# cvg/limap

Hardware: NVIDIA H100
Metric: 3D line candidates triangulated+scored/sec (higher is better)
Workload: dtype f64

## Files before the change

### limap_b200/csrc/engine.cu

```cuda
#include "engine.cuh"
#include <cub/device/device_radix_sort.cuh>
#include <cub/device/device_scan.cuh>
#include <algorithm>
#include <cstdlib>
#include <memory>
#include <set>

M3h quat_to_R(const double q_in[4]) {
  double n = std::sqrt(q_in[0] * q_in[0] + q_in[1] * q_in[1] + q_in[2] * q_in[2] + q_in[3] * q_in[3]);
  double q[4];
  if (n == 0) { q[0] = 1; q[1] = q_in[1]; q[2] = q_in[2]; q[3] = q_in[3]; }
  else for (int i = 0; i < 4; ++i) q[i] = q_in[i] / n;
  const double w = q[0], x = q[1], y = q[2], z = q[3];
  const double tx = 2 * x, ty = 2 * y, tz = 2 * z, twx = tx * w, twy = ty * w, twz = tz * w;
  const double txx = tx * x, txy = ty * x, txz = tz * x, tyy = ty * y, tyz = tz * y, tzz = tz * z;
  M3h R;
  R.m[0] = 1 - (tyy + tzz); R.m[1] = txy - twz; R.m[2] = txz + twy;
  R.m[3] = txy + twz; R.m[4] = 1 - (txx + tzz); R.m[5] = tyz - twx;
  R.m[6] = txz - twy; R.m[7] = tyz + twx; R.m[8] = 1 - (txx + tyy);
  return R;
}

void make_view(int model_id, const double *kv, const double *qv, const double *t, lm::ViewD &d) {
  const double fx = kv[0], fy = kv[1], cx = kv[2], cy = kv[3];
// ... 622 lines not shown
  p.ranges_flag = c->ranges_flag;
  for (int i = 0; i < 3; ++i) { p.rlo[i] = c->rlo[i]; p.rhi[i] = c->rhi[i]; }
  p.l2d = to_dev<double>(g.linker2d);
  {
    lm_linker_config l3 = g.linker3d;
    l3.use_angle = 1; l3.use_overlap = 0; l3.use_perp = 0; l3.use_innerseg = 0; l3.use_scaleinv = 1;
    p.l3d = to_dev<double>(l3);
  }
  {
    const double kPi = 3.14159265358979323846;
    const double t3 = p.l3d.th_angle, t2 = p.l2d.th_angle;
    p.cos_th3d_f = (t3 >= 90.0) ? -1.0f : (float)(std::cos(t3 * kPi / 180.0) - 4e-6);
    const double c2 = (t2 >= 90.0) ? 0.0 : std::cos(t2 * kPi / 180.0);
    p.cos2_th2d = c2 * c2;
    p.th_perp2_2d = p.l2d.th_perp * p.l2d.th_perp;
    const double ta = p.line_tri_angle_threshold, tsn = p.sensitivity_threshold;
    p.tri_poly_ok = (ta > 0.0 && ta < 90.0);
    p.sens_poly_ok = (tsn > 0.0 && tsn < 90.0);
    p.sin2_tri = std::sin(ta * kPi / 180.0) * std::sin(ta * kPi / 180.0);
    p.sin2_sens = std::sin(tsn * kPi / 180.0) * std::sin(tsn * kPi / 180.0);
    p.fast_forms = (p.l2d.use_innerseg || getenv("LIMAP_B200_REFERENCE_FORMS")) ? 0 : 1;
    p.inv_sig_a3 = 1.0 / (p.l3d.th_angle * p.l3d.mult);
    p.inv_sig_s3 = 1.0 / (p.l3d.th_scaleinv * p.l3d.mult);
    p.inv_sig_a2 = 1.0 / (p.l2d.th_angle * p.l2d.mult);
    p.inv_sig_p2 = 1.0 / (p.l2d.th_perp * p.l2d.mult);
    p.q_cut3 = -2.0 * std::log(p.l3d.score_th) * (1.0 + 1e-9);
    p.q_cut3_lo = -2.0 * std::log(p.l3d.score_th) * (1.0 - 1e-9);
    p.q_cut2 = -2.0 * std::log(p.l2d.score_th) * (1.0 + 1e-9);
    p.q_cut2_lo = -2.0 * std::log(p.l2d.score_th) * (1.0 - 1e-9);
    p.inv_smart_den2 = 1.0 / (p.l2d.th_smartoverlap - p.l2d.th_overlap);
  }
  int nbits = 1;
  while (((int64_t)1 << nbits) < c->n_nodes) ++nbits;
  c->sorted_key = c->d_key2.as<uint32_t>();
  c->sorted_val = c->d_val2.as<uint32_t>();
  p.row_ng = c->sorted_val;
  const int n_groups = exhaustive ? 1 : (int)std::max<int64_t>(1, std::min<int64_t>(c->pipeline_groups, n_rows >> 16));
  c->node_kernel_ms_acc = 0;
  int bg0 = 0, gv0 = vb;
  const int64_t n_shard_nodes = c->node_end - c->node_begin;
  if (!c->outside_shard_clean && (c->node_begin > 0 || c->node_end < c->n_nodes)) {
    if (c->node_begin > 0) {
      CU(cudaMemsetAsync(c->d_nodes.p, 0, sizeof(lm::NodeRecord) * c->node_begin, s));
      CU(cudaMemsetAsync(c->d_node_row_off.p, 0, 4 * c->node_begin, s));
    }
    if (c->node_end < c->n_nodes) {
      CU(cudaMemsetAsync(c->d_nodes.as<lm::NodeRecord>() + c->node_end, 0, sizeof(lm::NodeRecord) * (c->n_nodes - c->node_end), s));
      CU(cudaMemsetAsync(c->d_node_row_off.as<uint32_t>() + c->node_end + 1, 0, 4 * (c->n_nodes - c->node_end), s));
    }
    c->outside_shard_clean = true;
  }
  const bool fast_kernel = p.fast_forms && !p.use_endpoints_triangulation;
  const size_t smem_limit = (size_t)std::max(0, c->max_smem_optin - 1024);
  int cap = c->cap_hint > 0 ? c->cap_hint : 224;
  if (exhaustive && c->cap_hint == 0) {
    int64_t mr = 0, cur = 0;
    int cur_src = -1;
    for (int i = 0; i < nb; ++i) {
      if (blk[i].src_view != cur_src) { cur_src = blk[i].src_view; cur = 0; }
      cur += c->line_off[blk[i].ng_view + 1] - c->line_off[blk[i].ng_view];
      mr = std::max(mr, cur);
    }
    if (mr * ns > 65535) return fail(LM_ERR_INVALID, "more than 65535 candidates possible for one 2D line");
    cap = 32;
    while (cap < mr * ns) cap += 32;
  }
  while ((int)c->evk.size() < 2 * n_groups) {
    cudaEvent_t e;
    CU(cudaEventCreate(&e));
    c->evk.push_back(e);
  }
  while ((int)c->evp.size() < n_groups) {
    cudaEvent_t e;
    CU(cudaEventCreateWithFlags(&e, cudaEventDisableTiming));
    c->evp.push_back(e);
  }
  std::vector<int> group_has_kernel(n_groups, 0);
  CU(c->d_nvalid.ensure(4 * (n_shard_nodes + 2)));
  CU(c->d_local_off.ensure(4 * (n_shard_nodes + 2)));
  CU(c->d_edge_off.ensure(4 * (n_shard_nodes + 2)));
  CU(c->d_edge_ng.ensure(4 * std::max<int64_t>(n_rows * ns, 1)));
  for (int g = 0; g < n_groups; ++g) {
    int bg1 = nb, gv1 = ve;
    if (g + 1 < n_groups) {
      const double tg = (g + 1.0) / n_groups;
      const int64_t target = (int64_t)((double)n_rows * (tg * tg * (3.0 - 2.0 * tg)));
      bg1 = bg0;
      while (bg1 < nb && row_off[bg1] < target) ++bg1;
      while (bg1 < nb && bg1 > 0 && blk[bg1].src_view == blk[bg1 - 1].src_view) ++bg1;
      gv1 = (bg1 < nb) ? blk[bg1].src_view : ve;
    }
    const int64_t rb = row_off[bg0], re = row_off[bg1];
    const int64_t node_lo = c->line_off[gv0], node_hi = c->line_off[gv1];
    if (!exhaustive && re > rb) {
      int64_t need = 0;
      for (int b2 = bg0; b2 < bg1; ++b2) need = std::max(need, pair_off[b2] + blk[b2].n_rows);
      for (const auto &ch : c->chunks)
        if (ch.row_end >= need) { CU(cudaStreamWaitEvent(sp, ch.ev, 0)); break; }
    }
    unsigned int *d_max_rows = c->d_scalars.as<unsigned int>() + 16 + g;
    if (re > rb) {
      if (exhaustive)
        lm::launch_expand_exhaustive(c->d_blk_row_off.as<int64_t>(), c->d_blk_src.as<int32_t>(), c->d_blk_ng.as<int32_t>(),
                                     nb, c->d_line_off.as<int64_t>(), n_rows, c->d_key.as<uint32_t>(),
                                     c->d_val.as<uint32_t>(), sp);
      else
        lm::launch_expand_rows(c->d_pairs.as<int32_t>(), c->d_blk_row_off.as<int64_t>(), c->d_blk_src.as<int32_t>(),
                               c->d_blk_ng.as<int32_t>(), c->d_blk_pair_off.as<int64_t>(), nb,
                               c->d_line_off.as<int64_t>(), rb, re, c->d_key.as<uint32_t>(), c->d_val.as<uint32_t>(),
                               d_err, sp);
      ++launches;
      cub::DoubleBuffer<uint32_t> dk(c->d_key.as<uint32_t>() + rb, c->d_key2.as<uint32_t>() + rb);
      cub::DoubleBuffer<uint32_t> dv(c->d_val.as<uint32_t>() + rb, c->d_val2.as<uint32_t>() + rb);
      CU(cub_call(c->d_sort_tmp, [&](void *t, size_t &b) {
        return cub::DeviceRadixSort::SortPairs(t, b, dk, dv, (int)(re - rb), 0, nbits, sp);
      }));
      launches += (nbits + 7) / 8 + 1;
      if (dk.Current() != c->d_key2.as<uint32_t>() + rb) {
// ... 20 lines not shown
      p.cap = cap;
      grid = (int)std::min<int64_t>(n_group_nodes, (int64_t)c->sm_count * 4);
      p.slab_stride = (int64_t)((smem + 255) / 256 * 256);
      CU(c->d_slab.ensure((size_t)p.slab_stride * std::max(grid, 1)));
      p.slab = c->d_slab.as<char>();
      smem = 0;
    }
    if (n_group_nodes > 0) {
      CU(cudaEventRecord(c->evk[2 * g], s));
      CU(lm::launch_tri_node_kernel(p, grid, 128, smem, s));
      CU(cudaEventRecord(c->evk[2 * g + 1], s));
      group_has_kernel[g] = 1;
      ++launches;
      {
        cudaStream_t so = c->out_stream;
        CU(cudaStreamWaitEvent(so, c->evk[2 * g + 1], 0));
        uint32_t *nv = c->d_nvalid.as<uint32_t>() + (node_lo - c->node_begin);
        lm::launch_extract_nvalid(p.nodes, node_lo, n_group_nodes, nv, so);
        CU(cub_call(c->d_scan_tmp, [&](void *t, size_t &b) {
          return cub::DeviceScan::ExclusiveSum(t, b, nv, c->d_local_off.as<uint32_t>(), (int)(n_group_nodes + 1), so);
        }));
        lm::launch_group_edges(p.row_state, p.row_ng, p.node_row_off, c->d_local_off.as<uint32_t>(),
                               c->d_scalars.as<unsigned int>() + 80, g, c->node_begin, node_lo, n_group_nodes, ns,
                               c->d_edge_off.as<uint32_t>(), c->d_edge_ng.as<uint32_t>(), so);
        launches += 4;
      }
      if (c->node_sink) {
        CU(cudaMemcpyAsync(c->node_sink + sizeof(lm::NodeRecord) * node_lo, c->d_nodes.as<lm::NodeRecord>() + node_lo,
                           sizeof(lm::NodeRecord) * n_group_nodes, cudaMemcpyDeviceToHost, c->out_stream));
      }
    }
    bg0 = bg1;
    gv0 = gv1;
  }
  p.node_begin = c->node_begin;
  p.node_end = c->node_end;
  CU(cudaGetLastError());
  CU(cudaEventRecord(c->ev_run_begin, c->out_stream));
  CU(cudaStreamWaitEvent(s, c->ev_run_begin, 0));
  CU(cudaEventRecord(c->ev1, s));
  unsigned int *hs = c->h_pin;
  CU(cudaMemcpyAsync(hs, c->d_scalars.p, 512, cudaMemcpyDeviceToHost, s));
  CU(cudaStreamSynchronize(s));
  CU(cudaStreamSynchronize(c->copy_stream));
  CU(cudaStreamSynchronize(c->out_stream));
  c->stats.n_kernel_launches += launches;
  if (hs[1] == 1)
    return fail(LM_ERR_INVALID, "IndexError! Out-of-index matches exist (line_id >= number of lines of the image). "
                                "Please make sure you are reusing the correct descriptors and matches.");
  if (hs[1] == 2) return fail(LM_ERR_INVALID, "IndexError! Out-of-index neighbor line id in matches.");
  int max_rows_all = 0;
  for (int g = 0; g < n_groups; ++g) max_rows_all = std::max(max_rows_all, (int)hs[16 + g]);
  if ((int64_t)max_rows_all * ns > 65535) return fail(LM_ERR_INVALID, "more than 65535 candidates possible for one 2D line");
  int need_cap = 32;
  while (need_cap < max_rows_all * ns) need_cap += 32;
  c->cap_hint = need_cap;
  if (hs[2] != 0) {
    if (c->run_retry) { c->run_retry = 0; return fail(LM_ERR_STATE, "node staging overflow after resizing"); }
    c->run_retry = 1;
    const int rc2 = lm_tri_run(c);
    c->run_retry = 0;
    return rc2;
  }
  float ms = 0;
  CU(cudaEventElapsedTime(&ms, c->ev0, c->ev1));
  for (int g = 0; g < n_groups; ++g)
    if (group_has_kernel[g]) {
      float msk = 0;
      CU(cudaEventElapsedTime(&msk, c->evk[2 * g], c->evk[2 * g + 1]));
      c->node_kernel_ms_acc += msk;
    }
  c->stats.max_rows_per_node = max_rows_all;
  c->stats.last_node_kernel_ms = c->node_kernel_ms_acc;
  const unsigned long long *cnt = reinterpret_cast<const unsigned long long *>(hs + 4);
  c->stats.n_rows = n_rows;
  c->stats.n_candidates = (int64_t)cnt[0];
  c->stats.n_valid_edges = (int64_t)cnt[1];
  c->stats.n_pairs_gated = (int64_t)cnt[2];
  c->stats.n_pairs_exact = (int64_t)cnt[3];
  c->stats.last_run_ms = ms;
  c->ran = true;
  return LM_OK;
}

int lm_tri_get_stats(lm_ctx *c, lm_tri_stats *out) {
  if (!c || !out) return fail(LM_ERR_INVALID, "NULL argument");
  *out = c->stats;
  return LM_OK;
}

int lm_tri_get_best(lm_ctx *c, int32_t img_id, double *out_line, int32_t *out_ng, int32_t *out_ncand) {
  if (!c) return fail(LM_ERR_INVALID, "ctx is NULL");
  int rc = ensure_ran(c);
  if (rc) return rc;
  if ((rc = fetch_nodes(c))) return rc;
  auto it = c->id2view.find(img_id);
  if (it == c->id2view.end()) return fail(LM_ERR_INVALID, "unknown image id");
  const int v = it->second;
  for (int64_t n = c->line_off[v]; n < c->line_off[v + 1]; ++n) {
    const lm::NodeRecord &r = c->h_nodes[n];
    const int64_t l = n - c->line_off[v];
    for (int k = 0; k < 9; ++k) out_line[10 * l + k] = r.line[k];
    out_line[10 * l + 9] = r.score;
    out_ng[2 * l] = r.n_cand ? c->img_ids[r.ng_view] : 0;
    out_ng[2 * l + 1] = r.ng_line;
    if (out_ncand) out_ncand[l] = r.n_cand;
  }
  return LM_OK;
}
// ... 162 lines not shown
```

### limap_b200/csrc/tri_kernels.cu

```cuda
#include "tri_kernels.cuh"
#include <algorithm>
#include <cstdio>

namespace lm {

#ifndef LM_TRI_MIN_BLOCKS
#define LM_TRI_MIN_BLOCKS 4
#endif
static constexpr int kThreads = 128;
static constexpr int kWarps = kThreads / 32;
#ifndef LM_TRI_TMA
#define LM_TRI_TMA 0
#endif
#ifndef LM_KFLUSH
#define LM_KFLUSH 64
#endif
static constexpr int kFlush = LM_KFLUSH;
static constexpr int kListExtra = kFlush + 32;
static constexpr int kCandBytes = 17 * 8 + 48 + 8;

size_t tri_smem_bytes(int cap, bool fast) {
  if (fast) return (size_t)cap * (20 * 8 + kWarps * 8 + 32 + 8 + 4 + 2 + kWarps * 2);
  return (size_t)cap * kCandBytes + (size_t)kWarps * 2 * (cap + kListExtra) * 4 + (size_t)kWarps * cap * 2;
}

struct __align__(16) GateRec {
  float dx, dy, dz, lims2;
  float sx, sy, sz, lime2;
  float ex, ey, ez, pad;
};

struct __align__(16) GateRecF {
  float dx, dy, dz, lam_e;
  float lam_s;
  float lim_s, lim_e;
  int img;
};

struct Slab {
  double *sx, *sy, *sz, *ex, *ey, *ez, *dx, *dy, *dz, *zs, *ze, *unc, *q0, *q1, *q2, *q3, *score;
  double *izs2, *ize2, *inb;
  GateRec *gate;
  uint32_t *ng, *row;
  uint32_t *list;
  uint16_t *list0;
  GateRecF *gatef;
  float *slam;
  uint16_t *sidx;
  double *psc;
  uint16_t *pent;
  LM_D void carve(char *base, int cap, bool fast) {
    if (fast) { carve_fast(base, cap); return; }
    gatef = nullptr; slam = nullptr; sidx = nullptr; psc = nullptr; pent = nullptr;
    double *d = reinterpret_cast<double *>(base);
    sx = d; sy = sx + cap; sz = sy + cap; ex = sz + cap; ey = ex + cap; ez = ey + cap;
    dx = ez + cap; dy = dx + cap; dz = dy + cap; zs = dz + cap; ze = zs + cap; unc = ze + cap;
    q0 = unc + cap; q1 = q0 + cap; q2 = q1 + cap; q3 = q2 + cap; score = q3 + cap;
    double *nx = score + cap;
    izs2 = ize2 = inb = nullptr;
    if (fast) { izs2 = nx; ize2 = izs2 + cap; inb = ize2 + cap; nx = inb + cap; }
    gate = reinterpret_cast<GateRec *>(nx);
    ng = reinterpret_cast<uint32_t *>(gate + cap);
    row = ng + cap;
    list = row + cap;
    list0 = reinterpret_cast<uint16_t *>(list + (size_t)kWarps * (fast ? 1 : 2) * (cap + kListExtra));
  }
  LM_D void carve_fast(char *base, int cap) {
    double *d = reinterpret_cast<double *>(base);
    sx = d; sy = sx + cap; sz = sy + cap; ex = sz + cap; ey = ex + cap; ez = ey + cap;
    dx = ez + cap; dy = dx + cap; dz = dy + cap; zs = dz + cap; ze = zs + cap; unc = ze + cap;
    q0 = unc + cap; q1 = q0 + cap; q2 = q1 + cap; q3 = q2 + cap; score = q3 + cap;
    izs2 = score + cap; ize2 = izs2 + cap; inb = ize2 + cap;
    psc = inb + cap;
    gatef = reinterpret_cast<GateRecF *>(psc + (size_t)kWarps * cap);
    ng = reinterpret_cast<uint32_t *>(gatef + cap);
    row = ng + cap;
    slam = reinterpret_cast<float *>(row + cap);
    sidx = reinterpret_cast<uint16_t *>(slam + cap);
    pent = sidx + cap;
    gate = nullptr; list = nullptr; list0 = nullptr;
  }
};

LM_D uint32_t smem_u32(const void *p) { return (uint32_t)__cvta_generic_to_shared(p); }
LM_D void mbar_init(unsigned long long *bar, int count) {
  asm volatile("mbarrier.init.shared::cta.b64 [%0], %1;" ::"r"(smem_u32(bar)), "r"(count) : "memory");
  asm volatile("fence.mbarrier_init.release.cluster;" ::: "memory");
}
LM_D void mbar_arrive_expect_tx(unsigned long long *bar, uint32_t bytes) {
  asm volatile("mbarrier.arrive.expect_tx.shared::cta.b64 _, [%0], %1;" ::"r"(smem_u32(bar)), "r"(bytes) : "memory");
}
LM_D void bulk_copy_g2s(void *dst_smem, const void *src_gmem, uint32_t bytes, unsigned long long *bar) {
  asm volatile("cp.async.bulk.shared::cluster.global.mbarrier::complete_tx::bytes [%0], [%1], %2, [%3];" ::"r"(smem_u32(dst_smem)),
               "l"(src_gmem), "r"(bytes), "r"(smem_u32(bar))
               : "memory");
}
LM_D void mbar_wait(unsigned long long *bar, uint32_t parity) {
  uint32_t done = 0;
  while (!done) {
    asm volatile("{\n .reg .pred p;\n mbarrier.try_wait.parity.shared::cta.b64 p, [%1], %2;\n selp.u32 %0, 1, 0, p;\n}"
                 : "=r"(done)
                 : "r"(smem_u32(bar)), "r"(parity)
                 : "memory");
  }
}

struct Cand {
  vec3<double> s, e;
  double zs, ze, unc;
  double lam_s, lam_e;
};

LM_D double4 ld_seg(const double4 *p) {
  const double2 a = __ldg(reinterpret_cast<const double2 *>(p));
  const double2 b = __ldg(reinterpret_cast<const double2 *>(p) + 1);
  return make_double4(a.x, a.y, b.x, b.y);
}
LM_D double deg_from_cos_abs(double c) { return acos(fabs(c)) * consts<double>::rad2deg(); }

LM_D bool triangulate_point(const ViewD &v1, const ViewD &v2, vec3<double> n1e, vec3<double> n2e, vec3<double> C1,
                            vec3<double> C2, vec3<double> &out) {
  double a00 = dot(n1e, n1e), a01 = -dot(n1e, n2e), a10 = -dot(n2e, n1e), a11 = dot(n2e, n2e);
  double b0 = dot(n1e, C2 - C1), b1 = dot(n2e, C1 - C2);
  double r0, r1;
  if (a00 >= a11) {
    double l10 = a10 / a00, d1 = a11 - l10 * a01, y1 = b1 - l10 * b0;
    r1 = y1 / d1;
    r0 = (b0 - a01 * r1) / a00;
  } else {
    double l01 = a01 / a11, d0 = a00 - l01 * a10, y0 = b0 - l01 * b1;
    r0 = y0 / d0;
    r1 = (b1 - a10 * r0) / a11;
  }
// ... 191 lines not shown
  return true;
}

LM_D double pair_score(const TriParams &p, const seg<vec3<double>> &Li, vec3<double> di, double zsi, double zei,
                       const Slab &sl, int j, uint32_t vj) {
  const LinkerDev<double> &c3 = p.l3d;
  double score3 = 1.0;
  {
    double cs = fabs(di.x * sl.dx[j] + di.y * sl.dy[j] + di.z * sl.dz[j]);
    double angle = acos(cs) * consts<double>::rad2deg();
    score3 = smin(score3, thresh0(expscore(angle, c3.th_angle * c3.mult), c3.score_th));
    if (score3 < c3.score_th) return 0.0;
    vec3<double> sj = mk3(sl.sx[j], sl.sy[j], sl.sz[j]), ej = mk3(sl.ex[j], sl.ey[j], sl.ez[j]);
    double ds = norm(Li.s - sj), de = norm(Li.e - ej);
    double dist = smax(ds / (zsi + consts<double>::eps()), de / (zei + consts<double>::eps()));
    score3 = smin(score3, thresh0(expscore(dist, c3.th_scaleinv * c3.mult), c3.score_th));
    if (score3 == 0.0) return 0.0;
  }
  const ViewD &v = p.views[vj];
  seg<vec2<double>> a, b;
  a.s = dehom(proj_h(v.P, Li.s));
  a.e = dehom(proj_h(v.P, Li.e));
  b.s = mk2(sl.q0[j], sl.q1[j]);
  b.e = mk2(sl.q2[j], sl.q3[j]);
  double score2 = linker_score<double, vec2<double>>(p.l2d, a, b, 1.0, false, 0.0, 0.0);
  if (score2 == 0.0) return 0.0;
  return smin(score3, score2);
}

LM_D double asin2_over_t(double t) {
  double r = 0.017069849551821746;
  r = fma(r, t, 0.019089950090498877);
  r = fma(r, t, 0.02154247840073658);
  r = fma(r, t, 0.02456910759753428);
  r = fma(r, t, 0.028377319275152094);
  r = fma(r, t, 0.03328204112517838);
  r = fma(r, t, 0.03978243978243978);
  r = fma(r, t, 0.04871319157033443);
  r = fma(r, t, 0.06156806156806157);
  r = fma(r, t, 0.08126984126984127);
  r = fma(r, t, 0.11428571428571428);
  r = fma(r, t, 0.17777777777777778);
  r = fma(r, t, 0.3333333333333333);
  r = fma(r, t, 1.0);
  return r;
}
LM_D double angle2_deg(double t, double abs_cos) {
  const double k = consts<double>::rad2deg();
  if (t <= 0.0625) return t * asin2_over_t(t) * (k * k);
  const double a = acos(abs_cos) * k;
  return a * a;
}

LM_D double pair_score_fast(const TriParams &p, const Slab &sl, int i, int j, uint32_t vj) {
  const double EPS = consts<double>::eps();
  const LinkerDev<double> &c3 = p.l3d;
  const LinkerDev<double> &c2 = p.l2d;
  const vec3<double> si = mk3(sl.sx[i], sl.sy[i], sl.sz[i]), ei = mk3(sl.ex[i], sl.ey[i], sl.ez[i]);
  double Q = 0.0;
  {
    const vec3<double> di = mk3(sl.dx[i], sl.dy[i], sl.dz[i]), dj = mk3(sl.dx[j], sl.dy[j], sl.dz[j]);
    const vec3<double> cr = mk3(__dmul_rn(di.y, dj.z) - __dmul_rn(di.z, dj.y), __dmul_rn(di.z, dj.x) - __dmul_rn(di.x, dj.z),
                                __dmul_rn(di.x, dj.y) - __dmul_rn(di.y, dj.x));
    double a2 = angle2_deg(dot(cr, cr), fabs(dot(di, dj)));
    if (!(dot(di, di) * dot(dj, dj) > 0.5)) a2 = 8100.0;
    if (a2 == a2) Q = a2 * (p.inv_sig_a3 * p.inv_sig_a3);
    const vec3<double> ds = si - mk3(sl.sx[j], sl.sy[j], sl.sz[j]), de = ei - mk3(sl.ex[j], sl.ey[j], sl.ez[j]);
    const double r2 = fmax(dot(ds, ds) * sl.izs2[i], dot(de, de) * sl.ize2[i]);
    Q = fmax(Q, r2 * p.inv_sig_s3 * p.inv_sig_s3);
    if (Q > p.q_cut3) return 0.0;
  }
  const ViewD &v = p.views[vj];
  const vec3<double> hs = proj_h(v.P, si), he = proj_h(v.P, ei);
  const double ws = 1.0 / (hs.z + EPS), we = 1.0 / (he.z + EPS);
  const vec2<double> as = mk2(hs.x * ws, hs.y * ws), ae = mk2(he.x * we, he.y * we);
  const vec2<double> bs = mk2(sl.q0[j], sl.q1[j]), be = mk2(sl.q2[j], sl.q3[j]);
  const vec2<double> va = ae - as, vb = be - bs;
  const double na2 = dot(va, va), nb2 = dot(vb, vb);
  const double dab = dot(va, vb);
  const double ina = 1.0 / na2, inb = sl.inb[j];
  double Q2 = 0.0;
  double ang2 = 0.0;
  if (c2.use_angle) {
    if (dab * dab < p.cos2_th2d * na2 * nb2 * (1.0 - 1e-9)) return 0.0;
    if (na2 > 0.0 && nb2 > 0.0) {
      const double cr = va.x * vb.y - va.y * vb.x;
      const double t = cr * cr * (ina * inb);
      ang2 = angle2_deg(t, (t <= 0.0625) ? 0.0 : fabs(dab) / sqrt(na2 * nb2));
    } else {
      ang2 = 8100.0;
    }
    if (ang2 == ang2) Q2 = ang2 * (p.inv_sig_a2 * p.inv_sig_a2);
  }
  double bio = 0.0;
  if (c2.use_overlap) {
    double p1 = dot(as - bs, vb) * inb, p2 = dot(ae - bs, vb) * inb;
    if (p1 > p2) { const double t = p1; p1 = p2; p2 = t; }
    const double o1 = smin(p2, 1.0) - smax(p1, 0.0);
    double r1 = dot(bs - as, va) * ina, r2 = dot(be - as, va) * ina;
    if (r1 > r2) { const double t = r1; r1 = r2; r2 = t; }
    const double o2 = smin(r2, 1.0) - smax(r1, 0.0);
    bio = smax(o1, o2);
    if (!(bio > c2.th_overlap)) return 0.0;
  }
  if (c2.use_angle && c2.use_overlap && c2.use_smartangle && bio < c2.th_smartoverlap) {
    double ratio = (c2.th_smartoverlap - bio) * p.inv_smart_den2;
    ratio = smin(ratio, 1.0);
    const double sig = (c2.th_angle - ratio * (c2.th_angle - c2.th_smartangle)) * c2.mult;
    if (ang2 == ang2) Q2 = fmax(Q2, ang2 / (sig * sig));
  }
  if (c2.use_perp) {
    const vec2<double> d0 = as - bs, d1 = ae - bs, d2 = bs - as, d3 = be - as;
    const double t0 = dot(d0, vb), t1 = dot(d1, vb), t2 = dot(d2, va), t3 = dot(d3, va);
    double m = fmax(dot(d0, d0) - t0 * t0 * inb, 0.0);
    m = fmax(m, dot(d1, d1) - t1 * t1 * inb);
    m = fmax(m, dot(d2, d2) - t2 * t2 * ina);
    m = fmax(m, dot(d3, d3) - t3 * t3 * ina);
    Q2 = fmax(Q2, m * p.inv_sig_p2 * p.inv_sig_p2);
  }
  if (Q2 > p.q_cut2) return 0.0;
  if (Q < p.q_cut3_lo && Q2 < p.q_cut2_lo) return exp(-fmax(Q, Q2) * 0.5);
  const double e3 = exp(-Q * 0.5), e2 = exp(-Q2 * 0.5);
  if (e3 < c3.score_th || e2 < c2.score_th) return 0.0;
  return smin(e3, e2);
}


LM_D bool gate3d(const GateRec &r, const GateRec *g, float cos_th) {
  const float4 a = *reinterpret_cast<const float4 *>(&g->dx);
  const float cs = fabsf(r.dx * a.x + r.dy * a.y + r.dz * a.z);
  if (cs < cos_th) return false;
  const float4 b = *reinterpret_cast<const float4 *>(&g->sx);
  const float ax = r.sx - b.x, ay = r.sy - b.y, az = r.sz - b.z;
  if (ax * ax + ay * ay + az * az > r.lims2) return false;
  const float4 c = *reinterpret_cast<const float4 *>(&g->ex);
  const float bx = r.ex - c.x, by = r.ey - c.y, bz = r.ez - c.z;
  return !(bx * bx + by * by + bz * bz > r.lime2);
}

LM_D bool gate3d_rest(const GateRec &r, const GateRec *g, float cos_th) {
  const float4 a = *reinterpret_cast<const float4 *>(&g->dx);
  if (fabsf(r.dx * a.x + r.dy * a.y + r.dz * a.z) < cos_th) return false;
  const float4 c = *reinterpret_cast<const float4 *>(&g->ex);
  const float bx = r.ex - c.x, by = r.ey - c.y, bz = r.ez - c.z;
  return !(bx * bx + by * by + bz * bz > r.lime2);
}

LM_D bool gate2d(const TriParams &p, const seg<vec3<double>> &Li, const Slab &sl, int j, uint32_t vj) {
  const LinkerDev<double> &c = p.l2d;
  const ViewD &v = p.views[vj];
  const vec2<double> as = dehom(proj_h(v.P, Li.s)), ae = dehom(proj_h(v.P, Li.e));
  const vec2<double> bs = mk2(sl.q0[j], sl.q1[j]), be = mk2(sl.q2[j], sl.q3[j]);
  const vec2<double> va = ae - as, vb = be - bs;
  const double na2 = dot(va, va), nb2 = dot(vb, vb);
  const double REL = 1e-9;
  if (c.use_angle) {
    const double d = dot(va, vb);
    if (d * d < p.cos2_th2d * na2 * nb2 * (1.0 - REL)) return false;
  }
  if (c.use_overlap) {
    double p1 = dot(as - bs, vb) / nb2, p2 = dot(ae - bs, vb) / nb2;
    if (p1 > p2) { const double t = p1; p1 = p2; p2 = t; }
    const double o1 = smin(p2, 1.0) - smax(p1, 0.0);
    double r1 = dot(bs - as, va) / na2, r2 = dot(be - as, va) / na2;
    if (r1 > r2) { const double t = r1; r1 = r2; r2 = t; }
    const double o2 = smin(r2, 1.0) - smax(r1, 0.0);
    const double bio = smax(o1, o2);
    if (bio < c.th_overlap - REL * (1.0 + fabs(c.th_overlap))) return false;
  }
  if (c.use_perp) {
    const vec2<double> d0 = as - bs, d1 = ae - bs, d2 = bs - as, d3 = be - as;
    const double t0 = dot(d0, vb), t1 = dot(d1, vb), t2 = dot(d2, va), t3 = dot(d3, va);
    double m = dot(d0, d0) - t0 * t0 / nb2;
    m = fmax(m, dot(d1, d1) - t1 * t1 / nb2);
    m = fmax(m, dot(d2, d2) - t2 * t2 / na2);
    m = fmax(m, dot(d3, d3) - t3 * t3 / na2);
    if (m > p.th_perp2_2d * (1.0 + REL) + REL) return false;
  }
  return true;
}

template <bool SLAB, bool VP, bool FAST>
__global__ void __launch_bounds__(kThreads, LM_TRI_MIN_BLOCKS) tri_node_kernel(const __grid_constant__ TriParams p) {
  constexpr int NS = VP ? 3 : 1;
  extern __shared__ __align__(16) unsigned char smem_raw[];
  __shared__ int s_wtot[kWarps];
  __shared__ int s_nvalid;
  __shared__ int s_next_row;
  __shared__ __align__(8) unsigned long long s_mbar;
  uint32_t mbar_parity = 0;
  if constexpr (FAST && !SLAB && (LM_TRI_TMA || VP)) {
    if (threadIdx.x == 0) mbar_init(&s_mbar, 1);
    __syncthreads();
  }
  const int tid = threadIdx.x, lane = tid & 31, warp = tid >> 5;
  const unsigned lt_mask = (1u << lane) - 1u;
  Slab sl;
  if (SLAB) sl.carve(p.slab + (int64_t)blockIdx.x * p.slab_stride, p.cap, FAST);
  else sl.carve(reinterpret_cast<char *>(smem_raw), p.cap, FAST);
  uint32_t *list1 = FAST ? nullptr : sl.list + (size_t)(warp * 2) * (p.cap + kListExtra);
  uint32_t *list2 = FAST ? nullptr : list1 + p.cap + kListExtra;
  uint16_t *list0 = FAST ? nullptr : sl.list0 + (size_t)warp * p.cap;
  unsigned long long n1_total = 0, n2_total = 0;

  for (int64_t node = p.node_begin + blockIdx.x; node < p.node_end; node += gridDim.x) {
    const uint32_t r0 = p.node_row_off[node], r1 = p.node_row_off[node + 1];
    const int nrows = (int)(r1 - r0);
    NodeRecord *rec = &p.nodes[node];
    if (nrows == 0 || nrows * NS > p.cap) {
      if (tid < 9) rec->line[tid] = (tid == 8) ? -1.0 : 0.0;
      if (tid == 9) { rec->score = 0.0; rec->ng_view = 0; rec->ng_line = 0; rec->n_cand = 0; rec->n_valid = 0; }
      if (nrows != 0 && tid == 10) *p.overflow = 1;
      continue;
    }
    const ViewD *sviews = nullptr;
    const uint8_t *slot_of_row = nullptr;
    int n_stage = 0;
    if constexpr (FAST && !SLAB && (LM_TRI_TMA || VP)) {
      const int stage_off = p.cap * 4;
      ViewD *sv = reinterpret_cast<ViewD *>(reinterpret_cast<char *>(sl.psc) + stage_off);
      uint8_t *slots = reinterpret_cast<uint8_t *>(sl.sidx);
      const int stage_cap = min(255, (int)(((size_t)kWarps * p.cap * 8 - stage_off) / sizeof(ViewD)));
      int carry = 0;
      for (int base = 0; base < nrows; base += kThreads) {
        const int r = base + tid;
        uint32_t view = 0;
        int flag = 0;
        if (r < nrows) {
          view = __ldg(&p.row_ng[r0 + r]) >> 16;
          flag = (r == 0) || ((__ldg(&p.row_ng[r0 + r - 1]) >> 16) != view);
        }
        int incl = flag;
#pragma unroll
        for (int d = 1; d < 32; d <<= 1) {
          const int o = __shfl_up_sync(0xffffffffu, incl, d);
          if (lane >= d) incl += o;
        }
        if (lane == 31) s_wtot[warp] = incl;
        __syncthreads();
        int woff = 0, tot = 0;
#pragma unroll
        for (int w = 0; w < kWarps; ++w) {
          if (w < warp) woff += s_wtot[w];
          tot += s_wtot[w];
        }
        const int slot = carry + woff + incl - 1;
        if (r < nrows) slots[r] = (uint8_t)min(slot, 255);
        if (flag && slot < stage_cap) bulk_copy_g2s(sv + slot, p.views + view, (uint32_t)sizeof(ViewD), &s_mbar);
        carry += tot;
        __syncthreads();
      }
      n_stage = min(carry, stage_cap);
      if (tid == 0) mbar_arrive_expect_tx(&s_mbar, (uint32_t)(n_stage * sizeof(ViewD)));
      sviews = sv;
      slot_of_row = slots;
    }
    const uint32_t v1i = p.node_view[node];
    const ViewD &v1 = p.views[v1i];
    Src src;
    src.l1 = ld_seg(&p.segs[node]);
    {
      double dx = src.l1.x - src.l1.z, dy = src.l1.y - src.l1.w;
      src.ok = !(sqrt(dx * dx + dy * dy) <= p.min_length_2d);
      src.w1s = mat3_mul_h(v1.M, src.l1.x, src.l1.y);
      src.w1e = mat3_mul_h(v1.M, src.l1.z, src.l1.w);
      src.ray1s = normalized(src.w1s);
      src.ray1e = normalized(src.w1e);
      src.C1 = mk3(v1.C[0], v1.C[1], v1.C[2]);
      src.n1 = normalized(cross(src.w1s, src.w1e));
    }
    if constexpr (FAST && !SLAB && (LM_TRI_TMA || VP)) {
      mbar_wait(&s_mbar, mbar_parity);
      mbar_parity ^= 1u;
    }
    int count = 0;
    for (int base = 0; base < nrows; base += kThreads) {
      const int r = base + tid;
      Cand cs[NS];
      bool oks[NS];
#pragma unroll
      for (int k = 0; k < NS; ++k) oks[k] = false;
      double4 l2 = make_double4(0, 0, 0, 0);
      uint32_t ng = 0;
      if (r < nrows && src.ok) {
        ng = __ldg(&p.row_ng[r0 + r]);
        const uint32_t ngv = ng >> 16, ngl = ng & 0xffffu;
        if (VP) {
          const double4 l2v = ld_seg(&p.segs[p.line_off[ngv] + ngl]);
          const double ddx = l2v.x - l2v.z, ddy = l2v.y - l2v.w;
          if (!(sqrt(ddx * ddx + ddy * ddy) <= p.min_length_2d) && !p.disable_vp) {
            const ViewD *v2q = &p.views[ngv];
            if constexpr (FAST && !SLAB && (LM_TRI_TMA || VP)) {
              const int slot = slot_of_row[r];
              if (slot < n_stage) v2q = &sviews[slot];
            }
            const ViewD &v2 = *v2q;
            const vec3<double> c2s = mat3_mul_h(v2.M, l2v.x, l2v.y), c2e = mat3_mul_h(v2.M, l2v.z, l2v.w);
            const int lab1 = p.vp_label[node];
            if (lab1 >= 0) {
              const double *vp = p.vps + 3 * (p.vp_off[v1i] + lab1);
              oks[0] = gen_vp_candidate(p, v1, v2, src, c2s, c2e, normalized(mat3_mul(v1.M, mk3(vp[0], vp[1], vp[2]))), cs[0]);
            }
            const int lab2 = p.vp_label[p.line_off[ngv] + ngl];
            if (lab2 >= 0) {
              const double *vp = p.vps + 3 * (p.vp_off[ngv] + lab2);
              oks[1] = gen_vp_candidate(p, v1, v2, src, c2s, c2e, normalized(mat3_mul(v1.M, mk3(vp[0], vp[1], vp[2]))), cs[1]);
            }
          }
          l2 = l2v;
        }
        const ViewD *v2p = &p.views[ngv];
        if constexpr (FAST && !SLAB && (LM_TRI_TMA || VP)) {
          const int slot = slot_of_row[r];
          if (slot < n_stage) v2p = &sviews[slot];
        }
        oks[NS - 1] = gen_candidate<!FAST>(p, v1, *v2p, src, ngv, ngl, cs[NS - 1], l2);
      }
      int cnt = 0;
#pragma unroll
      for (int k = 0; k < NS; ++k) {
        if (r < nrows) p.row_state[(int64_t)(r0 + r) * NS + k] = 0;
        cnt += oks[k];
      }
      int incl = cnt;
#pragma unroll
      for (int d = 1; d < 32; d <<= 1) {
        const int o = __shfl_up_sync(0xffffffffu, incl, d);
        if (lane >= d) incl += o;
      }
      if (lane == 31) s_wtot[warp] = incl;
      __syncthreads();
      int woff = 0, tot = 0;
#pragma unroll
      for (int w = 0; w < kWarps; ++w) {
        if (w < warp) woff += s_wtot[w];
        tot += s_wtot[w];
      }
      int idx = count + woff + incl - cnt;
#pragma unroll
      for (int k = 0; k < NS; ++k) {
        if (!oks[k]) continue;
        const Cand &c = cs[k];
        const vec3<double> dr = c.e - c.s;
        const double dn2 = dot(dr, dr);
        const vec3<double> d = (dn2 > 0.0) ? dr * (1.0 / sqrt(dn2)) : dr;
        sl.sx[idx] = c.s.x; sl.sy[idx] = c.s.y; sl.sz[idx] = c.s.z;
        sl.ex[idx] = c.e.x; sl.ey[idx] = c.e.y; sl.ez[idx] = c.e.z;
        sl.dx[idx] = d.x; sl.dy[idx] = d.y; sl.dz[idx] = d.z;
        sl.zs[idx] = c.zs; sl.ze[idx] = c.ze; sl.unc[idx] = c.unc;
        sl.q0[idx] = l2.x; sl.q1[idx] = l2.y; sl.q2[idx] = l2.z; sl.q3[idx] = l2.w;
        if (FAST) {
          const double zs1 = c.zs + consts<double>::eps(), ze1 = c.ze + consts<double>::eps();
          const double qx = l2.z - l2.x, qy = l2.w - l2.y;
          sl.izs2[idx] = 1.0 / (zs1 * zs1); sl.ize2[idx] = 1.0 / (ze1 * ze1); sl.inb[idx] = 1.0 / (qx * qx + qy * qy);
        }
        sl.ng[idx] = ng;
        sl.row[idx] = (uint32_t)r * NS + k;
        if (FAST) {
          const double rad = fmax(fabs(c.lam_s), fabs(c.lam_e));
          const double ls = p.l3d.th_scaleinv * (c.zs + consts<double>::eps()) * 1.005 + 1e-5 * rad;
          const double le = p.l3d.th_scaleinv * (c.ze + consts<double>::eps()) * 1.005 + 1e-5 * rad;
          GateRecF g;
          g.dx = (float)d.x; g.dy = (float)d.y; g.dz = (float)d.z; g.lam_e = (float)c.lam_e;
          g.lam_s = (float)c.lam_s; g.lim_s = (float)(ls * 1.000001); g.lim_e = (float)(le * 1.000001);
          g.img = (int)(ng >> 16);
          sl.gatef[idx] = g;
          reinterpret_cast<float *>(sl.psc)[idx] = g.lam_s;
        } else {
          const vec3<double> rs = c.s - src.C1, re = c.e - src.C1;
          const double rad = sqrt(fmax(dot(rs, rs), dot(re, re)));
          const double ls = p.l3d.th_scaleinv * (c.zs + consts<double>::eps()) * 1.005 + 1e-5 * rad;
          const double le = p.l3d.th_scaleinv * (c.ze + consts<double>::eps()) * 1.005 + 1e-5 * rad;
          GateRec g;
          g.dx = (float)d.x; g.dy = (float)d.y; g.dz = (float)d.z; g.lims2 = (float)(ls * ls * 1.000001);
          g.sx = (float)rs.x; g.sy = (float)rs.y; g.sz = (float)rs.z; g.lime2 = (float)(le * le * 1.000001);
          g.ex = (float)re.x; g.ey = (float)re.y; g.ez = (float)re.z;
          g.pad = 0.f;
          sl.gate[idx] = g;
        }
        ++idx;
      }
      count += tot;
      __syncthreads();
    }
    const int C = count;
    if (tid == 0) { s_nvalid = 0; s_next_row = 0; }
    __syncthreads();
    if constexpr (FAST) {
      const unsigned FULL = 0xffffffffu;
      {
        float *ltmp = reinterpret_cast<float *>(sl.psc);
        const int C4 = (C + 3) & ~3;
        if (tid < C4 - C) ltmp[C + tid] = __int_as_float(0x7f800000);
        __syncthreads();
        for (int i = tid; i < C; i += kThreads) {
          const float li = ltmp[i];
          int r = 0;
          for (int j4 = 0; j4 < C4; j4 += 4) {
            const float4 v = *reinterpret_cast<const float4 *>(ltmp + j4);
            r += (v.x < li) || (v.x == li && j4 < i);
            r += (v.y < li) || (v.y == li && j4 + 1 < i);
            r += (v.z < li) || (v.z == li && j4 + 2 < i);
            r += (v.w < li) || (v.w == li && j4 + 3 < i);
          }
          sl.slam[r] = li;
          sl.sidx[r] = (uint16_t)i;
        }
// ... 50 lines not shown
                int rank = 0;
                while (m) {
                  const int t = __ffs((int)m) - 1;
                  m &= m - 1;
                  rank += __shfl_sync(FULL, j, t) < j;
                }
                if (ok) pent[fill + rank] = (uint16_t)j;
              }
            } else {
              uint16_t *tmp = reinterpret_cast<uint16_t *>(psc + fill);
              bool fits = true;
              for (int tb = 0; tb < W_r; tb += 32) {
                const int t = tb + lane;
                int j = 0;
                bool ok = false;
                if (t < W_r) {
                  j = sidx[lo_r + t];
                  const float4 gj = *reinterpret_cast<const float4 *>(&sl.gatef[j].dx);
                  const int imgj = sl.gatef[j].img;
                  ok = (imgj != __float_as_int(a1.w)) && !(fabsf(gj.w - a0.w) > a1.z) &&
                       !(fabsf(a0.x * gj.x + a0.y * gj.y + a0.z * gj.z) < p.cos_th3d_f);
                }
                const unsigned m = __ballot_sync(FULL, ok);
                if (fill + n_r + __popc(m) > p.cap) { fits = false; break; }
                if (ok) tmp[n_r + __popc(m & lt_mask)] = (uint16_t)j;
                n_r += __popc(m);
              }
              if (!fits) break;
              __syncwarp();
              for (int e = lane; e < n_r; e += 32) {
                const uint16_t v = tmp[e];
                int rank = 0;
                for (int x = 0; x < n_r; ++x) rank += tmp[x] < v;
                pent[fill + rank] = v;
              }
            }
            if (lane == rr) { off = fill; n = n_r; }
            fill += n_r;
          }
          const int ce = rr;
          n1_total += (unsigned long long)fill;
          __syncwarp();
          for (int fb = 0; fb < fill; fb += 32) {
            const int f = fb + lane;
            int r = cb;
#pragma unroll
            for (int step = 16; step >= 1; step >>= 1) {
              const int cand = r + step;
              const int v = __shfl_sync(FULL, off, cand & 31);
              if (cand < ce && v <= f) r = cand;
            }
            if (f < fill) {
              const int j = pent[f];
              psc[f] = pair_score_fast(p, sl, g0 + r, j, (uint32_t)sl.gatef[j].img);
            }
          }
          n2_total += (unsigned long long)fill;
          __syncwarp();
          if (lane >= cb && lane < ce) {
            double sum = 0.0, mx = 0.0;
            int cur = -1;
            for (int e = 0; e < n; ++e) {
              const int im = sl.gatef[pent[off + e]].img;
              const double sc = psc[off + e];
              if (im != cur) { sum += mx; cur = im; mx = sc; }
              else mx = (mx > sc) ? mx : sc;
            }
            sum += mx;
            sl.score[g0 + lane] = sum;
          }
          __syncwarp();
        }
      }
      __syncthreads();
    } else {
    for (int i = tid; i < C; i += kThreads) sl.score[i] = 0.0;
    if (tid < 32 && C + tid < ((C + 31) & ~31)) {
      GateRec z;
      z.dx = z.dy = z.dz = 0.f; z.lims2 = 0.f;
      z.sx = z.sy = z.sz = 3e18f; z.lime2 = 0.f;
      z.ex = z.ey = z.ez = 3e18f; z.pad = 0.f;
      sl.gate[C + tid] = z;
    }
    __syncthreads();
    bool more = true;
    while (more) {
      int n1 = 0;
      while (n1 < kFlush) {
        int i = 0;
        if (lane == 0) i = atomicAdd(&s_next_row, 1);
        i = __shfl_sync(0xffffffffu, i, 0);
        if (i >= C) { more = false; break; }
        const GateRec rf = sl.gate[i];
        const uint32_t vi = sl.ng[i] >> 16;
        int n0 = 0;
        for (int jb = 0; jb < C; jb += 32) {
          const int j = jb + lane;
          const float4 b = *reinterpret_cast<const float4 *>(&sl.gate[j].sx);
          const float ax = rf.sx - b.x, ay = rf.sy - b.y, az = rf.sz - b.z;
          const bool pass = !(ax * ax + ay * ay + az * az > rf.lims2);
          const unsigned bal = __ballot_sync(0xffffffffu, pass);
          if (pass) list0[n0 + __popc(bal & lt_mask)] = (uint16_t)j;
          n0 += __popc(bal);
        }
        __syncwarp();
        for (int kb = 0; kb < n0; kb += 32) {
          const int k = kb + lane;
          bool pass = false;
          int j = 0;
          if (k < n0) {
            j = list0[k];
            pass = (sl.ng[j] >> 16) != vi && gate3d_rest(rf, &sl.gate[j], p.cos_th3d_f);
          }
          const unsigned bal = __ballot_sync(0xffffffffu, pass);
          if (pass) list1[n1 + __popc(bal & lt_mask)] = ((uint32_t)i << 16) | (uint32_t)j;
          n1 += __popc(bal);
        }
        __syncwarp();
      }
      __syncwarp();
      n1_total += n1;
      if (n1 == 0) continue;
      int n2 = n1;
      uint32_t *listS = list1;
      if (!FAST) {
        n2 = 0;
        for (int kb = 0; kb < n1; kb += 32) {
          const int k = kb + lane;
          bool pass = false;
          uint32_t e = 0;
          if (k < n1) {
            e = list1[k];
            const int i = e >> 16, j = e & 0xffffu;
            seg<vec3<double>> Li;
            Li.s = mk3(sl.sx[i], sl.sy[i], sl.sz[i]);
            Li.e = mk3(sl.ex[i], sl.ey[i], sl.ez[i]);
            pass = gate2d(p, Li, sl, j, sl.ng[j] >> 16);
          }
          const unsigned bal = __ballot_sync(0xffffffffu, pass);
          if (pass) list2[n2 + __popc(bal & lt_mask)] = e;
          n2 += __popc(bal);
        }
        __syncwarp();
        listS = list2;
      }
      n2_total += n2;
      uint32_t carry_key = 0xffffffffu, cur_row = 0xffffffffu;
      double carry_max = 0.0, cur_sum = 0.0;
      for (int kb = 0; kb < n2; kb += 32) {
        const int k = kb + lane;
        double sc = 0.0;
        uint32_t key = 0xfffffffeu, row = 0xfffffffeu;
        if (k < n2) {
          const uint32_t e = listS[k];
          const int i = e >> 16, j = e & 0xffffu;
          const uint32_t vj = sl.ng[j] >> 16;
          row = (uint32_t)i;
          key = (row << 16) | vj;
          if (FAST) sc = pair_score_fast(p, sl, i, j, vj);
          else {
            seg<vec3<double>> Li;
            Li.s = mk3(sl.sx[i], sl.sy[i], sl.sz[i]);
            Li.e = mk3(sl.ex[i], sl.ey[i], sl.ez[i]);
            sc = pair_score(p, Li, mk3(sl.dx[i], sl.dy[i], sl.dz[i]), sl.zs[i], sl.ze[i], sl, j, vj);
          }
        }
        if (key == carry_key && carry_max > sc) sc = carry_max;
#pragma unroll
        for (int d = 1; d < 32; d <<= 1) {
          const double o = __shfl_up_sync(0xffffffffu, sc, d);
          const uint32_t ok = __shfl_up_sync(0xffffffffu, key, d);
          if (lane >= d && ok == key && o > sc) sc = o;
        }
        uint32_t knext = __shfl_down_sync(0xffffffffu, key, 1);
        if (lane == 31) {
          knext = 0xfffffffdu;
          if (k + 1 < n2) { const uint32_t e2 = listS[k + 1]; knext = (e2 & 0xffff0000u) | (sl.ng[e2 & 0xffffu] >> 16); }
        }
        const bool seg_end = (k < n2) && (knext != key);
        unsigned m = __ballot_sync(0xffffffffu, seg_end);
        while (m) {
          const int l = __ffs(m) - 1;
          const double v = __shfl_sync(0xffffffffu, sc, l);
          const uint32_t r = __shfl_sync(0xffffffffu, row, l);
          if (r != cur_row) {
            if (cur_row != 0xffffffffu && lane == 0) sl.score[cur_row] = cur_sum;
            cur_row = r;
            cur_sum = 0.0;
          }
          cur_sum += v;
          m &= m - 1;
        }
        const uint32_t k31 = __shfl_sync(0xffffffffu, key, 31);
        const double s31 = __shfl_sync(0xffffffffu, sc, 31);
        const bool end31 = __shfl_sync(0xffffffffu, (int)seg_end, 31);
        if (!end31 && kb + 31 < n2) { carry_key = k31; carry_max = s31; }
        else { carry_key = 0xffffffffu; carry_max = 0.0; }
      }
      if (cur_row != 0xffffffffu && lane == 0) sl.score[cur_row] = cur_sum;
      __syncwarp();
    }
    __syncthreads();
    }
    int nvalid_local = 0;
    for (int i = tid; i < C; i += kThreads) {
      const double sc = sl.score[i];
      bool valid = sc >= p.fullscore_th;
      if (valid && C > p.max_valid_conns) {
        int rank = 0;
        for (int k = 0; k < C; ++k) {
          const double sk = sl.score[k];
          rank += (sk > sc) || (sk == sc && k > i);
// ... 9 lines not shown
      }
    }
    if (nvalid_local) atomicAdd(&s_nvalid, nvalid_local);
    if (warp == 0) {
      double bs = -1.0;
      int bi = -1;
      for (int i = lane; i < C; i += 32) {
        const double sc = sl.score[i];
        if (sc > bs) { bs = sc; bi = i; }
      }
#pragma unroll
      for (int d = 16; d > 0; d >>= 1) {
        const double os = __shfl_down_sync(0xffffffffu, bs, d);
        const int oi = __shfl_down_sync(0xffffffffu, bi, d);
        if (oi >= 0 && (os > bs || (os == bs && (bi < 0 || oi < bi)))) { bs = os; bi = oi; }
      }
      bi = __shfl_sync(0xffffffffu, bi, 0);
      if (bi >= 0) {
        if (lane < 3) rec->line[lane] = (lane == 0) ? sl.sx[bi] : (lane == 1 ? sl.sy[bi] : sl.sz[bi]);
        else if (lane < 6) rec->line[lane] = (lane == 3) ? sl.ex[bi] : (lane == 4 ? sl.ey[bi] : sl.ez[bi]);
        else if (lane == 6) rec->line[6] = sl.zs[bi];
        else if (lane == 7) rec->line[7] = sl.ze[bi];
        else if (lane == 8) rec->line[8] = sl.unc[bi];
        else if (lane == 9) rec->score = sl.score[bi];
        else if (lane == 10) { rec->ng_view = (int32_t)(sl.ng[bi] >> 16); rec->ng_line = (int32_t)(sl.ng[bi] & 0xffffu); }
      } else {
        if (lane < 9) rec->line[lane] = (lane == 8) ? -1.0 : 0.0;
        if (lane == 9) rec->score = 0.0;
        if (lane == 10) { rec->ng_view = 0; rec->ng_line = 0; }
      }
    }
    __syncthreads();
    if (tid == 0) {
      rec->n_cand = C;
      rec->n_valid = s_nvalid;
      if (C) atomicAdd(&p.counters[0], (unsigned long long)C);
      if (s_nvalid) atomicAdd(&p.counters[1], (unsigned long long)s_nvalid);
    }
    __syncthreads();
  }
  if (lane == 0 && n1_total) {
    atomicAdd(&p.counters[2], n1_total);
    atomicAdd(&p.counters[3], n2_total);
  }
}

template <bool VP, bool FAST> static cudaError_t launch_tri_vf(const TriParams &p, int grid, size_t smem, cudaStream_t s) {
  if (p.use_slab) {
    tri_node_kernel<true, VP, FAST><<<grid, kThreads, 0, s>>>(p);
    return cudaGetLastError();
  }
  if (smem > 48 * 1024) {
    const cudaError_t e = cudaFuncSetAttribute(tri_node_kernel<false, VP, FAST>, cudaFuncAttributeMaxDynamicSharedMemorySize, (int)smem);
    if (e != cudaSuccess) return e;
  }
  tri_node_kernel<false, VP, FAST><<<grid, kThreads, smem, s>>>(p);
  return cudaGetLastError();
}
cudaError_t launch_tri_node_kernel(const TriParams &p, int grid, int block, size_t smem, cudaStream_t s) {
  (void)block;
  const bool fast = p.fast_forms && !p.use_endpoints_triangulation;
  if (p.use_vp) return fast ? launch_tri_vf<true, true>(p, grid, smem, s) : launch_tri_vf<true, false>(p, grid, smem, s);
  return fast ? launch_tri_vf<false, true>(p, grid, smem, s) : launch_tri_vf<false, false>(p, grid, smem, s);
}

__global__ void block_keys_kernel(const RawBlock *__restrict__ raw, int n_all, int vb, int ve, int exhaustive,
                                  uint32_t *__restrict__ key, uint32_t *__restrict__ val) {
  const int i = blockIdx.x * blockDim.x + threadIdx.x;
  if (i >= n_all) return;
  const RawBlock b = raw[i];
  const bool in = b.src_view >= vb && b.src_view < ve;
  key[i] = in ? (((uint32_t)b.src_view << 16) | (uint32_t)(exhaustive ? b.order : b.ng_view)) : 0xffffffffu;
  val[i] = (uint32_t)i;
}
__global__ void block_gather_kernel(const RawBlock *__restrict__ raw, const uint32_t *__restrict__ sorted_idx, int nb,
                                    int32_t *__restrict__ blk_src, int32_t *__restrict__ blk_ng,
                                    int64_t *__restrict__ blk_pair_off, int64_t *__restrict__ blk_rows) {
  const int i = blockIdx.x * blockDim.x + threadIdx.x;
  if (i > nb) return;
  if (i == nb) { blk_rows[i] = 0; return; }
  const RawBlock b = raw[sorted_idx[i]];
  blk_src[i] = b.src_view;
  blk_ng[i] = b.ng_view;
  blk_pair_off[i] = b.pair_off;
  blk_rows[i] = b.n_rows;
}
void launch_block_keys(const RawBlock *raw, int n_all, int vb, int ve, int exhaustive, uint32_t *key, uint32_t *val,
                       cudaStream_t s) {
  if (n_all <= 0) return;
  block_keys_kernel<<<(n_all + 255) / 256, 256, 0, s>>>(raw, n_all, vb, ve, exhaustive, key, val);
}
void launch_block_gather(const RawBlock *raw, const uint32_t *sorted_idx, int nb, int32_t *blk_src, int32_t *blk_ng,
                         int64_t *blk_pair_off, int64_t *blk_rows, cudaStream_t s) {
  block_gather_kernel<<<(nb + 1 + 255) / 256, 256, 0, s>>>(raw, sorted_idx, nb, blk_src, blk_ng, blk_pair_off, blk_rows);
}
__global__ void zero_words_kernel(unsigned int *p, int n) {
  const int i = blockIdx.x * blockDim.x + threadIdx.x;
  if (i < n) p[i] = 0u;
}
void launch_zero_words(void *d_dst, int n_words, cudaStream_t s) {
  zero_words_kernel<<<(n_words + 127) / 128, 128, 0, s>>>(static_cast<unsigned int *>(d_dst), n_words);
}

__global__ void expand_rows_kernel(const int32_t *__restrict__ pairs, const int64_t *__restrict__ blk_row_off,
                                   const int32_t *__restrict__ blk_src, const int32_t *__restrict__ blk_ng,
                                   const int64_t *__restrict__ blk_pair_off, int n_blocks,
// ... 301 lines not shown
```

Measured before the change: 2.434 billion.

## Shrink fast-path shared memory per candidate and raise occupancy of tri kernel

```diff
diff --git a/limap_b200/csrc/engine.cu b/limap_b200/csrc/engine.cu
--- a/limap_b200/csrc/engine.cu
+++ b/limap_b200/csrc/engine.cu
@@ -698,7 +698,9 @@
   }
   const bool fast_kernel = p.fast_forms && !p.use_endpoints_triangulation;
   const size_t smem_limit = (size_t)std::max(0, c->max_smem_optin - 1024);
-  int cap = c->cap_hint > 0 ? c->cap_hint : 224;
+  const int cap_step = fast_kernel ? 8 : 32;
+  auto round_cap = [&](int64_t n) { return (int)std::max<int64_t>(cap_step, (n + cap_step - 1) / cap_step * cap_step); };
+  int cap = c->cap_hint > 0 ? round_cap(c->cap_hint) : 224;
   if (exhaustive && c->cap_hint == 0) {
     int64_t mr = 0, cur = 0;
     int cur_src = -1;
@@ -708,8 +710,7 @@
       mr = std::max(mr, cur);
     }
     if (mr * ns > 65535) return fail(LM_ERR_INVALID, "more than 65535 candidates possible for one 2D line");
-    cap = 32;
-    while (cap < mr * ns) cap += 32;
+    cap = round_cap(mr * ns);
   }
   while ((int)c->evk.size() < 2 * n_groups) {
     cudaEvent_t e;
@@ -836,9 +837,7 @@
   int max_rows_all = 0;
   for (int g = 0; g < n_groups; ++g) max_rows_all = std::max(max_rows_all, (int)hs[16 + g]);
   if ((int64_t)max_rows_all * ns > 65535) return fail(LM_ERR_INVALID, "more than 65535 candidates possible for one 2D line");
-  int need_cap = 32;
-  while (need_cap < max_rows_all * ns) need_cap += 32;
-  c->cap_hint = need_cap;
+  c->cap_hint = round_cap((int64_t)max_rows_all * ns);
   if (hs[2] != 0) {
     if (c->run_retry) { c->run_retry = 0; return fail(LM_ERR_STATE, "node staging overflow after resizing"); }
     c->run_retry = 1;
diff --git a/limap_b200/csrc/tri_kernels.cu b/limap_b200/csrc/tri_kernels.cu
--- a/limap_b200/csrc/tri_kernels.cu
+++ b/limap_b200/csrc/tri_kernels.cu
@@ -5,7 +5,7 @@
 namespace lm {
 
 #ifndef LM_TRI_MIN_BLOCKS
-#define LM_TRI_MIN_BLOCKS 4
+#define LM_TRI_MIN_BLOCKS 5
 #endif
 static constexpr int kThreads = 128;
 static constexpr int kWarps = kThreads / 32;
@@ -20,7 +20,7 @@
 static constexpr int kCandBytes = 17 * 8 + 48 + 8;
 
 size_t tri_smem_bytes(int cap, bool fast) {
-  if (fast) return (size_t)cap * (20 * 8 + kWarps * 8 + 32 + 8 + 4 + 2 + kWarps * 2);
+  if (fast) return (size_t)cap * (16 * 8 + kWarps * 8 + 32 + 8 + 4 + 2 + kWarps * 2);
   return (size_t)cap * kCandBytes + (size_t)kWarps * 2 * (cap + kListExtra) * 4 + (size_t)kWarps * cap * 2;
 }
 
@@ -69,8 +69,7 @@
     double *d = reinterpret_cast<double *>(base);
     sx = d; sy = sx + cap; sz = sy + cap; ex = sz + cap; ey = ex + cap; ez = ey + cap;
     dx = ez + cap; dy = dx + cap; dz = dy + cap; zs = dz + cap; ze = zs + cap; unc = ze + cap;
-    q0 = unc + cap; q1 = q0 + cap; q2 = q1 + cap; q3 = q2 + cap; score = q3 + cap;
-    izs2 = score + cap; ize2 = izs2 + cap; inb = ize2 + cap;
+    score = unc + cap; izs2 = score + cap; ize2 = izs2 + cap; inb = ize2 + cap;
     psc = inb + cap;
     gatef = reinterpret_cast<GateRecF *>(psc + (size_t)kWarps * cap);
     ng = reinterpret_cast<uint32_t *>(gatef + cap);
@@ -78,7 +77,7 @@
     slam = reinterpret_cast<float *>(row + cap);
     sidx = reinterpret_cast<uint16_t *>(slam + cap);
     pent = sidx + cap;
-    gate = nullptr; list = nullptr; list0 = nullptr;
+    q0 = q1 = q2 = q3 = nullptr; gate = nullptr; list = nullptr; list0 = nullptr;
   }
 };
 
@@ -376,7 +375,8 @@
   return a * a;
 }
 
-LM_D double pair_score_fast(const TriParams &p, const Slab &sl, int i, int j, uint32_t vj) {
+LM_D double pair_score_fast(const TriParams &p, const Slab &sl, int i, int j, uint32_t ngj) {
+  const uint32_t vj = ngj >> 16;
   const double EPS = consts<double>::eps();
   const LinkerDev<double> &c3 = p.l3d;
   const LinkerDev<double> &c2 = p.l2d;
@@ -398,7 +398,8 @@
   const vec3<double> hs = proj_h(v.P, si), he = proj_h(v.P, ei);
   const double ws = 1.0 / (hs.z + EPS), we = 1.0 / (he.z + EPS);
   const vec2<double> as = mk2(hs.x * ws, hs.y * ws), ae = mk2(he.x * we, he.y * we);
-  const vec2<double> bs = mk2(sl.q0[j], sl.q1[j]), be = mk2(sl.q2[j], sl.q3[j]);
+  const double4 q = ld_seg(&p.segs[p.line_off[vj] + (ngj & 0xffffu)]);
+  const vec2<double> bs = mk2(q.x, q.y), be = mk2(q.z, q.w);
   const vec2<double> va = ae - as, vb = be - bs;
   const double na2 = dot(va, va), nb2 = dot(vb, vb);
   const double dab = dot(va, vb);
@@ -505,12 +506,14 @@
 }
 
 template <bool SLAB, bool VP, bool FAST>
-__global__ void __launch_bounds__(kThreads, LM_TRI_MIN_BLOCKS) tri_node_kernel(const __grid_constant__ TriParams p) {
+__global__ void __launch_bounds__(kThreads, (!SLAB && !VP && FAST) ? LM_TRI_MIN_BLOCKS : 4)
+    tri_node_kernel(const __grid_constant__ TriParams p) {
   constexpr int NS = VP ? 3 : 1;
   extern __shared__ __align__(16) unsigned char smem_raw[];
   __shared__ int s_wtot[kWarps];
   __shared__ int s_nvalid;
   __shared__ int s_next_row;
+  __shared__ Src s_src;
   __shared__ __align__(8) unsigned long long s_mbar;
   uint32_t mbar_parity = 0;
   if constexpr (FAST && !SLAB && (LM_TRI_TMA || VP)) {
@@ -581,9 +584,9 @@
     }
     const uint32_t v1i = p.node_view[node];
     const ViewD &v1 = p.views[v1i];
-    Src src;
-    src.l1 = ld_seg(&p.segs[node]);
-    {
+    if (tid == 0) {
+      Src src;
+      src.l1 = ld_seg(&p.segs[node]);
       double dx = src.l1.x - src.l1.z, dy = src.l1.y - src.l1.w;
       src.ok = !(sqrt(dx * dx + dy * dy) <= p.min_length_2d);
       src.w1s = mat3_mul_h(v1.M, src.l1.x, src.l1.y);
@@ -592,7 +595,10 @@
       src.ray1e = normalized(src.w1e);
       src.C1 = mk3(v1.C[0], v1.C[1], v1.C[2]);
       src.n1 = normalized(cross(src.w1s, src.w1e));
-    }
+      s_src = src;
+    }
+    __syncthreads();
+    const Src &src = s_src;
     if constexpr (FAST && !SLAB && (LM_TRI_TMA || VP)) {
       mbar_wait(&s_mbar, mbar_parity);
       mbar_parity ^= 1u;
@@ -646,6 +652,8 @@
         if (r < nrows) p.row_state[(int64_t)(r0 + r) * NS + k] = 0;
         cnt += oks[k];
       }
+      const double qx = l2.z - l2.x, qy = l2.w - l2.y;
+      const double nq2 = qx * qx + qy * qy;
       int incl = cnt;
 #pragma unroll
       for (int d = 1; d < 32; d <<= 1) {
@@ -672,11 +680,11 @@
         sl.ex[idx] = c.e.x; sl.ey[idx] = c.e.y; sl.ez[idx] = c.e.z;
         sl.dx[idx] = d.x; sl.dy[idx] = d.y; sl.dz[idx] = d.z;
         sl.zs[idx] = c.zs; sl.ze[idx] = c.ze; sl.unc[idx] = c.unc;
-        sl.q0[idx] = l2.x; sl.q1[idx] = l2.y; sl.q2[idx] = l2.z; sl.q3[idx] = l2.w;
         if (FAST) {
           const double zs1 = c.zs + consts<double>::eps(), ze1 = c.ze + consts<double>::eps();
-          const double qx = l2.z - l2.x, qy = l2.w - l2.y;
-          sl.izs2[idx] = 1.0 / (zs1 * zs1); sl.ize2[idx] = 1.0 / (ze1 * ze1); sl.inb[idx] = 1.0 / (qx * qx + qy * qy);
+          sl.izs2[idx] = 1.0 / (zs1 * zs1); sl.ize2[idx] = 1.0 / (ze1 * ze1); sl.inb[idx] = 1.0 / nq2;
+        } else {
+          sl.q0[idx] = l2.x; sl.q1[idx] = l2.y; sl.q2[idx] = l2.z; sl.q3[idx] = l2.w;
         }
         sl.ng[idx] = ng;
         sl.row[idx] = (uint32_t)r * NS + k;
@@ -833,7 +841,7 @@
             }
             if (f < fill) {
               const int j = pent[f];
-              psc[f] = pair_score_fast(p, sl, g0 + r, j, (uint32_t)sl.gatef[j].img);
+              psc[f] = pair_score_fast(p, sl, g0 + r, j, sl.ng[j]);
             }
           }
           n2_total += (unsigned long long)fill;
@@ -938,7 +946,7 @@
           const uint32_t vj = sl.ng[j] >> 16;
           row = (uint32_t)i;
           key = (row << 16) | vj;
-          if (FAST) sc = pair_score_fast(p, sl, i, j, vj);
+          if (FAST) sc = pair_score_fast(p, sl, i, j, sl.ng[j]);
           else {
             seg<vec3<double>> Li;
             Li.s = mk3(sl.sx[i], sl.sy[i], sl.sz[i]);
@@ -1054,6 +1062,11 @@
   }
   if (smem > 48 * 1024) {
     const cudaError_t e = cudaFuncSetAttribute(tri_node_kernel<false, VP, FAST>, cudaFuncAttributeMaxDynamicSharedMemorySize, (int)smem);
+    if (e != cudaSuccess) return e;
+  }
+  if constexpr (!VP && FAST) {
+    const cudaError_t e = cudaFuncSetAttribute(tri_node_kernel<false, VP, FAST>, cudaFuncAttributePreferredSharedMemoryCarveout,
+                                               (int)cudaSharedmemCarveoutMaxShared);
     if (e != cudaSuccess) return e;
   }
   tri_node_kernel<false, VP, FAST><<<grid, kThreads, smem, s>>>(p);
```

Result: faster. 2.593 billion (median of 6 runs) (+6.6%).
